# HyoKong/Cross-Resolution-Face-Recognition

Hardware: NVIDIA B200
Metric: fsrnet_train_images_per_sec (higher is better)
Workload: dtype bf16

## Files before the change

cross-resolution-face-recognition_b200/csrc/internal.h:

```cpp
#pragma once
#include <cuda_runtime.h>
#include <stddef.h>

#include "crfr.h"

#ifdef __cplusplus
#include <atomic>
#endif

enum {
  CRFR_OPT_ROWCONV_PAIR = 0,
  CRFR_OPT_WGRAD_STREAM,
  CRFR_OPT_NORM_BWD_STREAM,
  CRFR_OPT_NORM_FWD_STREAM,
  CRFR_OPT_FUSE_NORM_BWD,
  CRFR_OPT_COUNT
};
int crfr_opt(int id);

template <typename K>
inline int crfr_smem_attr(K kernel, int bytes, std::atomic<unsigned long long>& done) {
  int dev = 0;
  if (cudaGetDevice(&dev) != cudaSuccess) dev = -1;
  const unsigned long long bit = (dev >= 0 && dev < 64) ? 1ull << dev : 0ull;
// ... 18 lines not shown
  const float* rscale = nullptr;
  const float* sscale = nullptr;
};
struct crfr_pack_batch {
  crfr_pack_job job[CRFR_PACK_BATCH];
  int njobs;
};
int crfr_pack_weight_batch(const crfr_pack_job* jobs, int n, cudaStream_t st);

size_t crfr_norm_ws_bytes(int n, int hw, int c);
int crfr_norm_finalize(const float* partial, int n, int chunks, int hw, int c, float eps, float* stats,
                       cudaStream_t st);
int crfr_norm_bwd_finish(const float* partial, int chunks, const void* dsrc, int dsrc_ld, int recompute, const void* y,
                         int y_ld, const float* stats, const float* gamma, const float* beta, const float* alpha, int relu,
                         void* dy, int dy_ld, float* dgamma, float* dbeta, float* dalpha, int n, int hw, int c,
                         float* bstats, float* tot, int use_stream, cudaStream_t st);

int crfr_norm_stream_supported(int c, long long npix, const void* const* views, const int* lds, int count);
int crfr_norm_stream_parts(int n, int hw, int c);
int crfr_norm_bwd_reduce_stream(const void* da, int da_ld, const void* db, int db_ld, const void* y, int y_ld,
                                const float* stats, const float* gamma, const float* beta, const float* alpha, int relu,
                                const void* res, int res_ld, void* dz, int dz_ld, int n, int hw, int c, float* partial,
                                cudaStream_t st);
int crfr_norm_bwd_apply_stream(const void* dsrc, int dsrc_ld, int recompute, const void* y, int y_ld, const float* stats,
                               const float* partial, int parts, const float* bstats, const float* tot,
                               const float* gamma, const float* beta,
                               const float* alpha, int relu, void* dy, int dy_ld, float* dgamma, float* dbeta,
                               float* dalpha, int n, int hw, int c, cudaStream_t st);

int crfr_norm_fwd_stream(const void* y, int y_ld, const float* stats, const float* gamma, const float* beta,
                         const float* alpha, int relu, const void* res, int res_ld, void* out, int out_ld, int n, int hw,
                         int c, cudaStream_t st);

int crfr_loss_mse97_chan(const float* x, const float* t, int n, int c, int hw, float gscale, float* loss, void* dx,
                         int dx_ld, float* dchan, void* ws, size_t ws_bytes, cudaStream_t st);
int crfr_nchw_chansum(const float* g, int n, int c, int hw, float* out, void* ws, size_t ws_bytes, cudaStream_t st);

int crfr_direct_gather(int down, int n, int bh, int bw, int sh, int sw, int k, int stride, int pad, const void* src,
                       int src_ld, const void* w, int R, int s_pad, const float* bias, void* y, int y_ld,
                       float* y_nchw, cudaStream_t st);
int crfr_direct_wgrad(int n, int bh, int bw, int sh, int sw, int k, int stride, int pad, const void* small,
                      int small_ld, int A, const void* big, int big_ld, int B, float* G, void* ws, size_t ws_bytes, cudaStream_t st);
int crfr_colsum(const void* t, int ld, int c, long long npix, float* out, void* ws, size_t ws_bytes, cudaStream_t st);

struct TcGemm {
  const void* src; int n, h, w, k_total, src_ld;
  const void* wt;
  int ksize, pad, sign;
  int n_total, tile_n;
  void* out; int out_ld, out_f32;
  const float* bias;
  float* stat_ws = nullptr; size_t stat_ws_bytes = 0; int* stat_slots = nullptr;
  int stat_batch = 0;
};
int crfr_tc_gemm(const TcGemm& g, cudaStream_t st);
struct TcWgrad {
  const void* x; int n, h, w, cin, x_ld;
  const void* dy; int cout, dy_ld;
  int taps3x3;
  float* G;
  float* part = nullptr;
  size_t part_bytes = 0;
};
int crfr_tc_wgrad_raw(const TcWgrad& g, cudaStream_t st);
size_t crfr_tc_wgrad_part_bytes();

int crfr_tc_supported(int op, int h, int w, int cin, int cout, int k, int stride, int pad);
size_t crfr_tc_workspace_bytes(const crfr_conv_desc* d);
int crfr_tc_conv(const crfr_conv_desc* d, int dgrad, const void* src, const void* w_packed, const float* bias,
                 void* dst, float* stats, float eps, void* ws, size_t ws_bytes, cudaStream_t st, int batch_stats = 0);
int crfr_conv_fwd_bnstats(int engine, const crfr_conv_desc* d, const void* x, const void* w_packed, int cin_pad, void* y,
                          float* bn_stats, float eps, void* ws, size_t ws_bytes, cudaStream_t st);
int crfr_tc_wgrad(const crfr_conv_desc* d, const void* x, const void* dy, float* dw, void* ws, size_t ws_bytes,
                  cudaStream_t st);

int crfr_lowered_recipe(const crfr_conv_desc* d);
size_t crfr_lowered_ws_bytes(const crfr_conv_desc* d);
int crfr_lowered_fwd(const crfr_conv_desc* d, const void* x, const void* w_packed, int cin_pad, const float* bias,
                     void* y, float* y_nchw, void* ws, size_t ws_bytes, cudaStream_t st, float* stats = nullptr,
                     float eps = 0.f, int* stats_done = nullptr);
int crfr_lowered_dgrad(const crfr_conv_desc* d, const void* dy, const void* w_packed_t, int cout_pad, void* dx, void* ws,
                       size_t ws_bytes, cudaStream_t st);
int crfr_lowered_wgrad(const crfr_conv_desc* d, const void* x, const void* dy, float* dw, void* ws, size_t ws_bytes,
                       cudaStream_t st);
size_t crfr_lowered_dgrad_cin3_ws_bytes(const crfr_conv_desc* d);
int crfr_lowered_dgrad_cin3(const crfr_conv_desc* d, const void* dy, const void* w_packed_t, void* dx, void* ws,
                            size_t ws_bytes, cudaStream_t st);

int crfr_rowconv_supported(int h, int w, int cin, int cout, int k, int stride, int pad);
size_t crfr_rowconv_ws_bytes(int n, int h);
int crfr_rowconv_pair_supported(int n, int h);
size_t crfr_rowconv_pair_ws_bytes(int n, int h);
struct crfr_rowconv_fuse {
  const void* y; int y_ld;
  const void* db; int db_ld;
  const void* res; int res_ld;
  const float* stats; const float* gamma; const float* beta; const float* alpha; int relu;
  float* partial;
};
int crfr_rowconv_pair_parts(int n, int h, int plain = 0);
int crfr_rowconv_pair(const void* src, int src_ld, int n, int h, const void* w_packed, int flip, const float* bias,
                      void* dst, int dst_ld, float* stats, float eps, void* ws, size_t ws_bytes, cudaStream_t st,
                      const crfr_rowconv_fuse* fuse = nullptr);
int crfr_rowwgrad_supported(int h, int w, int cin, int cout, int k, int stride, int pad);
size_t crfr_rowwgrad_ws_bytes(int n, int h);
int crfr_rowwgrad(const void* x, int x_ld, const void* dy, int dy_ld, int n, int h, float* dw, void* ws,
// ... 4 lines not shown
```

cross-resolution-face-recognition_b200/csrc/lowered_conv.cu:

```cuda
#include "common.cuh"
#include "crfr.h"
#include "internal.h"

namespace {

template <int KS>
__global__ void im2col_small_kernel(const bf16* __restrict__ x, int h, int w, int oh, int ow, int stride, int pad, int sign,
                                    bf16* __restrict__ P, int kpad, int rows) {
  const int groups = kpad >> 3;
  const int idx = blockIdx.x * blockDim.x + threadIdx.x;
  if (idx >= ow * groups) return;
  const int ox = idx / groups, g = idx - ox * groups;
  const int k0 = g * 8, kmax = KS * KS * 3;
  for (int row = blockIdx.y; row < rows; row += gridDim.y) {
  const int n = row / oh, oy = row - n * oh;
  uint32_t out[4] = {0u, 0u, 0u, 0u};
  if (k0 < kmax) {
    const int t0 = k0 / 3;
    uint2 pv[4];
#pragma unroll
    for (int ti = 0; ti < 4; ++ti) {
      const int tap = t0 + ti;
      const int ky = tap / KS, kx = tap - ky * KS;
      const int y = oy * stride + sign * (ky - pad), xx = ox * stride + sign * (kx - pad);
// ... 130 lines not shown
  if (gy > (unsigned)rows) gy = (unsigned)rows;
  const dim3 grid(gx, gy);
  if (ks == 3) im2col_small_kernel<3><<<grid, 256, 0, st>>>(x, h, w, oh, ow, stride, pad, sign, P, kpad, rows);
  else if (ks == 7) im2col_small_kernel<7><<<grid, 256, 0, st>>>(x, h, w, oh, ow, stride, pad, sign, P, kpad, rows);
  else {
    crfr_set_error("im2col_small: kernel size %d not instantiated", ks);
    return CRFR_EUNSUPPORTED;
  }
  CRFR_COUNT_LAUNCH();
  CRFR_LAUNCH_CHECK();
  return CRFR_OK;
}

__global__ void col2im_small_kernel(const float* __restrict__ src, int src_ld, int C, int sh, int sw, int bh, int bw,
                                    int ks, int stride, int pad, int sgn, const float* __restrict__ bias,
                                    float* __restrict__ y_nchw, bf16* __restrict__ y, int y_ld, long long total) {
  long long i = (long long)blockIdx.x * blockDim.x + threadIdx.x;
  if (i >= total) return;
  const int X = (int)(i % bw);
  long long q = i / bw;
  const int Y = (int)(q % bh);
  const long long n = q / bh;
  float acc[4] = {0.f, 0.f, 0.f, 0.f};
#pragma unroll
  for (int c = 0; c < 4; ++c) acc[c] = (bias && c < C) ? bias[c] : 0.f;
  const int ky0 = sgn > 0 ? (Y + pad) % stride : ((pad - Y) % stride + stride) % stride;
  const int kx0 = sgn > 0 ? (X + pad) % stride : ((pad - X) % stride + stride) % stride;
  for (int ky = ky0; ky < ks; ky += stride) {
    const int ty = Y + sgn * (pad - ky);
    if (ty < 0) continue;
    const int sy = ty / stride;
    if (sy >= sh) continue;
    for (int kx = kx0; kx < ks; kx += stride) {
      const int tx = X + sgn * (pad - kx);
      if (tx < 0) continue;
      const int sx = tx / stride;
      if (sx >= sw) continue;
      const float* s = src + ((n * sh + sy) * sw + sx) * src_ld + (ky * ks + kx) * C;
#pragma unroll
      for (int c = 0; c < 4; ++c)
        if (c < C) acc[c] += s[c];
    }
  }
  if (y_nchw) {
#pragma unroll
    for (int c = 0; c < 4; ++c)
      if (c < C) y_nchw[(n * C + c) * ((long long)bh * bw) + (long long)Y * bw + X] = acc[c];
  }
  if (y) {
#pragma unroll
    for (int c = 0; c < 4; ++c)
      if (c < y_ld) y[i * y_ld + c] = __float2bfloat16_rn(c < C ? acc[c] : 0.f);
    for (int c = 4; c < y_ld; ++c) y[i * y_ld + c] = __float2bfloat16_rn(0.f);
  }
}

__global__ void __launch_bounds__(256)
col2im3_s1_kernel(const float* __restrict__ src, int h, int w, int sgn, const float* __restrict__ bias,
                  float* __restrict__ y_nchw, bf16* __restrict__ y, int y_ld) {
  constexpr int TH = 8, TW = 32, SH = TH + 2, SW = TW + 2, LD = 33;
  __shared__ float tile[SH * SW * LD];
  const int tiles_x = (w + TW - 1) / TW, tiles_y = h / TH;
  int b = blockIdx.x;
  const int tx0 = (b % tiles_x) * TW;
  b /= tiles_x;
  const int ty0 = (b % tiles_y) * TH;
  const long long n = b / tiles_y;
  const float* img = src + n * h * w * 32;
  for (int i = threadIdx.x; i < SH * SW * 8; i += 256) {
    const int px = i >> 3, q = i & 7;
    const int sy = ty0 - 1 + px / SW, sx = tx0 - 1 + px % SW;
    float4 v = make_float4(0.f, 0.f, 0.f, 0.f);
    if (sy >= 0 && sy < h && sx >= 0 && sx < w) v = *reinterpret_cast<const float4*>(img + ((long long)sy * w + sx) * 32 + q * 4);
    float* t = tile + px * LD + q * 4;
    t[0] = v.x; t[1] = v.y; t[2] = v.z; t[3] = v.w;
  }
  __syncthreads();
  const int ly = threadIdx.x >> 5, lx = threadIdx.x & 31;
  float acc[3];
#pragma unroll
  for (int c = 0; c < 3; ++c) acc[c] = bias ? bias[c] : 0.f;
#pragma unroll
  for (int ky = 0; ky < 3; ++ky)
#pragma unroll
    for (int kx = 0; kx < 3; ++kx) {
      const float* t = tile + ((ly + 1 + sgn * (1 - ky)) * SW + (lx + 1 + sgn * (1 - kx))) * LD + (ky * 3 + kx) * 3;
#pragma unroll
      for (int c = 0; c < 3; ++c) acc[c] += t[c];
    }
  const int Y = ty0 + ly, X = tx0 + lx;
  if (X >= w) return;
  if (y_nchw)
#pragma unroll
    for (int c = 0; c < 3; ++c) y_nchw[((n * 3 + c) * h + Y) * w + X] = acc[c];
  if (y) {
    const long long i = (n * h + Y) * w + X;
    for (int c = 0; c < y_ld; ++c) y[i * y_ld + c] = __float2bfloat16_rn(c < 3 ? acc[c] : 0.f);
  }
}

__device__ __forceinline__ void subpixel_of_tap(int k, int* phase, int* off) {
  const int p = (k + 2) & 3;
  *phase = p;
  *off = (p + 2 - k) / 4;
}

__global__ void deconv_subpixel_pack_kernel(const bf16* __restrict__ src, bf16* __restrict__ dst, int mode) {
  const int i = blockIdx.x * blockDim.x + threadIdx.x;
  if (i >= 49 * 64 * 64) return;
  const int s_ = i & 63, r = (i >> 6) & 63, tap = i >> 12;
  int py, dy, px, dx;
  subpixel_of_tap(tap / 7, &py, &dy);
  subpixel_of_tap(tap % 7, &px, &dx);
  const int t9 = (dy + 1) * 3 + (dx + 1), ph = py * 4 + px;
  if (mode == 0) dst[((size_t)t9 * 1024 + ph * 64 + r) * 64 + s_] = src[i];
  else dst[((size_t)t9 * 64 + r) * 1024 + ph * 64 + s_] = src[i];
}

__global__ void deconv_bias_kernel(const float* __restrict__ bias, float* __restrict__ big) {
  const int i = blockIdx.x * blockDim.x + threadIdx.x;
  if (i < 1024) big[i] = bias ? bias[i & 63] : 0.f;
}

__global__ void deconv_shuffle_kernel(bf16* __restrict__ y, int y_ld, bf16* __restrict__ all, int sh, int sw, int to_all,
                                      long long total) {
  const long long i = (long long)blockIdx.x * blockDim.x + threadIdx.x;
  if (i >= total) return;
  const int g = (int)(i & 7);
  long long p = i >> 3;
  const int X = (int)(p % (4 * sw));
  long long q = p / (4 * sw);
  const int Y = (int)(q % (4 * sh));
  const long long n = q / (4 * sh);
  const long long ai = ((n * sh + (Y >> 2)) * sw + (X >> 2)) * 1024 + ((Y & 3) * 4 + (X & 3)) * 64 + g * 8;
  uint4* py_ = reinterpret_cast<uint4*>(y + p * y_ld + g * 8);
  uint4* pa = reinterpret_cast<uint4*>(all + ai);
  if (to_all) *pa = *py_;
  else *py_ = *pa;
}

__global__ void deconv_subpixel_unpack_kernel(const float* __restrict__ G, float* __restrict__ dw) {
  const int i = blockIdx.x * blockDim.x + threadIdx.x;
  if (i >= 64 * 64 * 49) return;
  const int tap = i % 49, co = (i / 49) & 63, ci = i / (49 * 64);
  int py, dy, px, dx;
  subpixel_of_tap(tap / 7, &py, &dy);
  subpixel_of_tap(tap % 7, &px, &dx);
  const int t9 = (dy + 1) * 3 + (dx + 1), ph = py * 4 + px;
  dw[i] += G[((size_t)t9 * 64 + ci) * 1024 + ph * 64 + co];
}

__global__ void im2col_vec_kernel(const bf16* __restrict__ x, int x_ld, int C, int h, int w, int oh, int ow, int ks,
                                  int stride, int pad, bf16* __restrict__ P, long long total) {
  long long i = (long long)blockIdx.x * blockDim.x + threadIdx.x;
  if (i >= total) return;
  const int groups = C >> 3, T = ks * ks;
  const int g = (int)(i % groups);
  long long r = i / groups;
  const int tap = (int)(r % T);
  long long o = r / T;
  const int ox = (int)(o % ow);
  long long q = o / ow;
  const int oy = (int)(q % oh);
  const long long n = q / oh;
  const int ky = tap / ks, kx = tap - ky * ks;
  const int y = oy * stride + ky - pad, xx = ox * stride + kx - pad;
  uint4 v = make_uint4(0u, 0u, 0u, 0u);
  if (y >= 0 && y < h && xx >= 0 && xx < w)
    v = *reinterpret_cast<const uint4*>(x + ((n * h + y) * w + xx) * x_ld + g * 8);
// ... 217 lines not shown
      CRFR_COUNT_LAUNCH();
      CRFR_LAUNCH_CHECK();
      return CRFR_OK;
    }
    LAUNCH(col2im_small_kernel, pix, st, Q, 32, 3, d->h, d->w, d->h, d->w, 3, 1, 1, -1, bias, y_nchw, (bf16*)y,
           y ? d->out_ld : 0, pix);
    return CRFR_OK;
  }
  if (recipe == 4) {
    if (!y || y_nchw) {
      crfr_set_error("lowered conv: the transposed recipe produces the bf16 NHWC output only");
      return CRFR_EUNSUPPORTED;
    }
    const long long ipix = (long long)d->n * d->h * d->w, opix = (long long)d->n * d->oh * d->ow;
    TAKE(All, bf16, A, (size_t)ipix * 1024 * 2);
    TAKE(Wbig, bf16, A, (size_t)9 * 1024 * 64 * 2);
    TAKE(bbig, float, A, 1024 * 4);
    CRFR_CUDA(cudaMemsetAsync(Wbig, 0, (size_t)9 * 1024 * 64 * 2, st));
    LAUNCH(deconv_subpixel_pack_kernel, 49 * 64 * 64, st, (const bf16*)w_packed, Wbig, 0);
    LAUNCH(deconv_bias_kernel, 1024, st, bias, bbig);
    TcGemm g{x, d->n, d->h, d->w, 64, d->in_ld, Wbig, 3, 1, 1, 1024, 256, All, 1024, 0, bbig};
    CRFR_TRY(crfr_tc_gemm(g, st));
    LAUNCH(deconv_shuffle_kernel, opix * 8, st, (bf16*)y, d->out_ld, All, d->h, d->w, 0, opix * 8);
    return CRFR_OK;
  }
  crfr_set_error("lowered conv: no recipe for this shape");
  return CRFR_EUNSUPPORTED;
}

int crfr_lowered_dgrad(const crfr_conv_desc* d, const void* dy, const void* w_packed_t, int cout_pad, void* dx, void* ws,
                       size_t ws_bytes, cudaStream_t st) {
  const int recipe = crfr_lowered_recipe(d);
  Arena A{(uint8_t*)ws, ws_bytes, 0};
  const int T = d->k * d->k;
  if (recipe == 2) {
    const long long pix = (long long)d->n * d->h * d->w;
    TAKE(R, bf16, A, (size_t)pix * 64 * 2);
    TAKE(Wd, bf16, A, (size_t)64 * 64 * 2);
    CRFR_TRY(launch_im2col_small((const bf16*)dy, d->n, d->h, d->w, d->h, d->w, 3, 1, 1, -1, R, 64, st));
    LAUNCH(repack_tapmajor_kernel, 64 * 64, st, (const bf16*)w_packed_t, T, 64, 3, cout_pad, Wd, 64, 64);
    TcGemm g{R, d->n, d->h, d->w, 64, 64, Wd, 1, 0, 1, 64, 64, dx, d->in_ld, 0, nullptr};
    return crfr_tc_gemm(g, st);
  }
  if (recipe == 3) {
    const int kp = kpad_of(d);
    const long long opix = (long long)d->n * d->oh * d->ow, ipix = (long long)d->n * d->h * d->w;
    TAKE(dP, float, A, (size_t)opix * kp * 4);
    TAKE(Wd, bf16, A, (size_t)kp * d->cout * 2);
    CRFR_CUDA(cudaMemsetAsync(Wd, 0, (size_t)kp * d->cout * 2, st));
    CRFR_CHECK_ARG(cout_pad == d->cout, "lowered dgrad: cout_pad %d != cout %d", cout_pad, d->cout);
    CRFR_CUDA(cudaMemcpyAsync(Wd, w_packed_t, (size_t)T * 3 * d->cout * 2, cudaMemcpyDeviceToDevice, st));
    TcGemm g{dy, d->n, d->oh, d->ow, d->cout, d->out_ld, Wd, 1, 0, 1, kp, kp == 192 ? 192 : 0, dP, kp, 1, nullptr};
    CRFR_TRY(crfr_tc_gemm(g, st));
    LAUNCH(col2im_small_kernel, ipix, st, dP, kp, 3, d->oh, d->ow, d->h, d->w, d->k, d->stride, d->pad, 1, nullptr, nullptr,
           (bf16*)dx, d->in_ld, ipix);
    return CRFR_OK;
  }
  if (recipe == 5) {
    CRFR_CHECK_ARG(cout_pad == d->cout, "lowered dgrad: cout_pad %d != cout %d", cout_pad, d->cout);
    const int kc = T * d->cin;
    const long long opix = (long long)d->n * d->oh * d->ow, ipix = (long long)d->n * d->h * d->w;
    TAKE(dP, float, A, (size_t)opix * kc * 4);
    TcGemm g{dy, d->n, d->oh, d->ow, d->cout, d->out_ld, w_packed_t, 1, 0, 1, kc, 0, dP, kc, 1, nullptr};
    CRFR_TRY(crfr_tc_gemm(g, st));
    LAUNCH(col2im_vec_kernel, ipix * (d->cin / 8), st, dP, d->cin, d->oh, d->ow, d->h, d->w, d->k, d->stride, d->pad,
           (bf16*)dx, d->in_ld, ipix * (d->cin / 8));
    return CRFR_OK;
  }
  if (recipe == 4) {
    CRFR_CHECK_ARG(cout_pad == 64, "lowered dgrad: cout_pad %d != 64", cout_pad);
    const long long ipix = (long long)d->n * d->h * d->w, opix = (long long)d->n * d->oh * d->ow;
    TAKE(All, bf16, A, (size_t)ipix * 1024 * 2);
    TAKE(Wbig, bf16, A, (size_t)9 * 64 * 1024 * 2);
    LAUNCH(deconv_shuffle_kernel, opix * 8, st, (bf16*)const_cast<void*>(dy), d->out_ld, All, d->h, d->w, 1, opix * 8);
    CRFR_CUDA(cudaMemsetAsync(Wbig, 0, (size_t)9 * 64 * 1024 * 2, st));
    LAUNCH(deconv_subpixel_pack_kernel, 49 * 64 * 64, st, (const bf16*)w_packed_t, Wbig, 1);
    TcGemm g{All, d->n, d->h, d->w, 1024, 1024, Wbig, 3, 1, -1, 64, 64, dx, d->in_ld, 0, nullptr};
    return crfr_tc_gemm(g, st);
  }
  crfr_set_error("lowered dgrad: no recipe for this shape");
  return CRFR_EUNSUPPORTED;
}

size_t crfr_lowered_dgrad_cin3_ws_bytes(const crfr_conv_desc* d) {
  return (size_t)d->n * d->h * d->w * 32 * 4 + (size_t)32 * 64 * 2 + 4096;
}

int crfr_lowered_dgrad_cin3(const crfr_conv_desc* d, const void* dy, const void* w_packed_t, void* dx, void* ws,
                            size_t ws_bytes, cudaStream_t st) {
  if (crfr_lowered_recipe(d) != 1 || d->cout != 64 || d->out_ld != 64 || d->h % 8) {
    crfr_set_error("lowered dgrad (3-channel input): unsupported shape");
    return CRFR_EUNSUPPORTED;
  }
  Arena A{(uint8_t*)ws, ws_bytes, 0};
  const long long pix = (long long)d->n * d->h * d->w;
  TAKE(Q, float, A, (size_t)pix * 32 * 4);
  TAKE(Wq, bf16, A, (size_t)32 * 64 * 2);
  CRFR_CUDA(cudaMemsetAsync(Wq, 0, (size_t)32 * 64 * 2, st));
  CRFR_CUDA(cudaMemcpyAsync(Wq, w_packed_t, (size_t)27 * 64 * 2, cudaMemcpyDeviceToDevice, st));
  TcGemm g{dy, d->n, d->h, d->w, 64, d->out_ld, Wq, 1, 0, 1, 32, 32, Q, 32, 1, nullptr};
  CRFR_TRY(crfr_tc_gemm(g, st));
  col2im3_s1_kernel<<<(unsigned)(d->n * (d->h / 8) * ((d->w + 31) / 32)), 256, 0, st>>>(Q, d->h, d->w, 1, nullptr, nullptr,
                                                                                       (bf16*)dx, d->in_ld);
  CRFR_COUNT_LAUNCH();
  CRFR_LAUNCH_CHECK();
  return CRFR_OK;
}

int crfr_lowered_wgrad(const crfr_conv_desc* d, const void* x, const void* dy, float* dw, void* ws, size_t ws_bytes,
                       cudaStream_t st) {
  const int recipe = crfr_lowered_recipe(d);
  Arena A{(uint8_t*)ws, ws_bytes, 0};
  const int T = d->k * d->k;
  if (recipe == 1 || recipe == 3) {
    const int kp = kpad_of(d);
    const long long opix = (long long)d->n * d->oh * d->ow;
    TAKE(P, bf16, A, (size_t)opix * kp * 2);
    TAKE(G, float, A, (size_t)kp * d->cout * 4);
    CRFR_TRY(launch_im2col_small((const bf16*)x, d->n, d->h, d->w, d->oh, d->ow, d->k, d->stride, d->pad, 1, P, kp, st));
    CRFR_CUDA(cudaMemsetAsync(G, 0, (size_t)kp * d->cout * 4, st));
    TcWgrad g{P, d->n, d->oh, d->ow, kp, kp, dy, d->cout, d->out_ld, 0, G};
    A.rest(&g.part, &g.part_bytes);
    CRFR_TRY(crfr_tc_wgrad_raw(g, st));
    LAUNCH(unpack_lowered_kernel, (long long)d->cout * 3 * T, st, G, d->cout, dw, d->cout, 3, T, 0);
    return CRFR_OK;
  }
  if (recipe == 5) {
    const int kc = T * d->cin;
    const long long opix = (long long)d->n * d->oh * d->ow;
    TAKE(P, bf16, A, (size_t)opix * kc * 2);
// ... 38 lines not shown
```

cross-resolution-face-recognition_b200/csrc/tc_conv.cu:

```cuda
#include <cudaTypedefs.h>
#include <stdlib.h>

#include "common.cuh"
#include "crfr.h"
#include "internal.h"
#include "sm100.cuh"

using namespace sm100;

namespace {

int make_act_map(CUtensorMap* m, const void* ptr, int n, int h, int w, int c, int ld, int bw, int bh, int bn) {
  const unsigned long long dims[4] = {(unsigned long long)c, (unsigned long long)w, (unsigned long long)h,
                                      (unsigned long long)n};
  const unsigned long long strides[3] = {(unsigned long long)ld * 2, (unsigned long long)w * ld * 2,
                                         (unsigned long long)h * w * ld * 2};
  const unsigned int box[4] = {64, (unsigned int)bw, (unsigned int)bh, (unsigned int)bn};
  return crfr_tmap_encode_bf16(m, ptr, 4, dims, strides, box, "activation");
}

int make_weight_map(CUtensorMap* m, const void* ptr, long long rows, int kdim, int box_rows) {
  const unsigned long long dims[2] = {(unsigned long long)kdim, (unsigned long long)rows};
  const unsigned long long strides[1] = {(unsigned long long)kdim * 2};
  const unsigned int box[2] = {64, (unsigned int)box_rows};
  return crfr_tmap_encode_bf16(m, ptr, 2, dims, strides, box, "weights");
}

struct Tiling {
  int bw, bh, bn, tiles_x, tiles_y, tiles_n, rows;
};

bool make_tiling(int n, int h, int w, Tiling* t) {
  if (w >= 128) {
    t->bw = 128; t->bh = 1; t->bn = 1;
  } else {
    t->bw = w;
    t->bh = 128 / w;
    if (t->bh > h) t->bh = h;
    if (t->bh < 1) return false;
    t->bn = 128 / (t->bw * t->bh);
    if (t->bn < 1) t->bn = 1;
    if (t->bn > 256) return false;
  }
  t->rows = t->bw * t->bh * t->bn;
  t->tiles_x = (w + t->bw - 1) / t->bw;
  t->tiles_y = (h + t->bh - 1) / t->bh;
  t->tiles_n = (n + t->bn - 1) / t->bn;
  return t->rows <= 128 && t->rows >= 1;
}

struct ConvParams {
  int n, h, w;
  int kchunks, ksize, ntaps, pad, sign;
  int bw, bh, bn, tiles_x, tiles_y, rows;
  int total_tiles;
  int n_total;
  int out_ld;
  int out_f32;
  void* out;
  const float* bias;
  float* partial;
  int slots, gpt;
};

constexpr int kConvThreads = 192;
constexpr int kATileBytes = 128 * 128;

constexpr int kResidentIters = 9;
template <int N, int MODE = 0>
struct ConvCfg {
  static constexpr bool R = MODE == 1, T2 = MODE == 2;
  static constexpr int kBTileBytes = N * 128;
  static constexpr int kStageBytes = R ? 2 * kATileBytes : (T2 ? 2 : 1) * kATileBytes + kBTileBytes;
  static constexpr int kStages = (R || T2) ? 4 : (N <= 64) ? 8 : (N <= 128) ? 6 : 3;
  static constexpr int kAccBufs = T2 ? 4 : 2;
  static constexpr int kResidentBytes = R ? kResidentIters * kBTileBytes : 0;
  static constexpr int kTmemCols = (N <= 32) ? 32 : (N <= 64) ? 64 : (N <= 128) ? 128 : 256;
  static constexpr int kOutTiles = (N + 63) / 64;
  static constexpr int kOutBytes = kOutTiles * kATileBytes;
  static constexpr int kSmemBytes = kStages * kStageBytes + kResidentBytes + kOutBytes + 1024  + 256 ;
  static_assert(N % 32 == 0 && N <= 256 && kAccBufs * kTmemCols <= 512, "tile width");
  static_assert(kSmemBytes <= 232448, "shared memory budget");
};

template <int N, int MODE>
__global__ void __launch_bounds__(kConvThreads, 1)
tc_conv_kernel(const __grid_constant__ CUtensorMap tmA, const __grid_constant__ CUtensorMap tmB,
               const __grid_constant__ CUtensorMap tmY, ConvParams p) {
  using Cfg = ConvCfg<N, MODE>;
  constexpr bool R = Cfg::R, T2 = Cfg::T2;
  constexpr int kAB = Cfg::kAccBufs;
  extern __shared__ uint8_t smem_raw[];
  uint8_t* base = (uint8_t*)(((uintptr_t)smem_raw + 1023) & ~(uintptr_t)1023);
  uint8_t* sB = base + Cfg::kStages * Cfg::kStageBytes;
  uint8_t* sOut = sB + Cfg::kResidentBytes;
  uint64_t* full = (uint64_t*)(sOut + Cfg::kOutBytes);
  uint64_t* empty = full + Cfg::kStages;
  uint64_t* tmem_full = empty + Cfg::kStages;
  uint64_t* tmem_empty = tmem_full + kAB;
  uint64_t* w_full = tmem_empty + kAB;
  uint32_t* tmem_slot = (uint32_t*)(w_full + 1);

  const int warp = threadIdx.x >> 5, lane = threadIdx.x & 31;
  if (threadIdx.x == 0) {
    for (int s = 0; s < Cfg::kStages; ++s) {
      mbar_init(&full[s], 1);
      mbar_init(&empty[s], 1);
    }
    for (int b = 0; b < kAB; ++b) {
      mbar_init(&tmem_full[b], 1);
      mbar_init(&tmem_empty[b], 4);
    }
    mbar_init(w_full, 1);
    fence_barrier_init();
    prefetch_tmap(&tmA);
    prefetch_tmap(&tmB);
    prefetch_tmap(&tmY);
  }
  if (warp == 1) tmem_alloc<kAB * Cfg::kTmemCols>(tmem_slot);
  tc_fence_before();
  __syncthreads();
  tc_fence_after();
  const uint32_t tmem = *tmem_slot;

  const int iters = R ? 3 : p.ntaps * p.kchunks;
  const uint32_t a_bytes = (uint32_t)p.rows * 128u;
  const int ncol0 = blockIdx.y * N;
  const int my_tiles = (int)blockIdx.x < p.total_tiles ? (p.total_tiles - (int)blockIdx.x + (int)gridDim.x - 1) / (int)gridDim.x : 0;

  if (warp == 0) {
    const bool leader = elect_one();
    if (R && leader && my_tiles > 0) {
      mbar_expect_tx(w_full, (uint32_t)kResidentIters * Cfg::kBTileBytes);
      for (int tap = 0; tap < kResidentIters; ++tap)
        tma_load_2d(sB + tap * Cfg::kBTileBytes, &tmB, w_full, 0, tap * p.n_total + ncol0);
    }
    int g = 0;
    for (int i = 0; i < my_tiles; i += T2 ? 2 : 1) {
      int t = blockIdx.x + i * gridDim.x;
      const int tx = t % p.tiles_x; t /= p.tiles_x;
      const int ty = t % p.tiles_y; t /= p.tiles_y;
      const int x0 = tx * p.bw, y0 = ty * p.bh, n0 = t * p.bn;
      const bool has2 = T2 && i + 1 < my_tiles;
      int t1 = blockIdx.x + (has2 ? i + 1 : i) * gridDim.x;
      const int tx1 = t1 % p.tiles_x; t1 /= p.tiles_x;
      const int ty1 = t1 % p.tiles_y; t1 /= p.tiles_y;
      const int x1 = tx1 * p.bw, y1 = ty1 * p.bh, n1 = t1 * p.bn;
      for (int it = 0; it < iters; ++it, ++g) {
        const int s = g % Cfg::kStages;
        mbar_wait(&empty[s], ((g / Cfg::kStages) & 1) ^ 1);
        uint8_t* sa = base + s * Cfg::kStageBytes;
        if (R) {
          if (leader) {
            mbar_expect_tx(&full[s], (uint32_t)((p.bh + 2) * p.bw) * 128u);
            tma_load_4d(sa, &tmA, &full[s], 0, x0 + p.sign * (it - 1), y0 - 1, n0);
          }
          continue;
        }
        const int tap = it / p.kchunks, kc = it - tap * p.kchunks;
        const int ky = tap / p.ksize, kx = tap - ky * p.ksize;
        if (leader) {
          mbar_expect_tx(&full[s], (has2 ? 2u : 1u) * a_bytes + (uint32_t)Cfg::kBTileBytes);
          tma_load_4d(sa, &tmA, &full[s], kc * 64, x0 + p.sign * (kx - p.pad), y0 + p.sign * (ky - p.pad), n0);
          if (has2) tma_load_4d(sa + kATileBytes, &tmA, &full[s], kc * 64, x1 + p.sign * (kx - p.pad), y1 + p.sign * (ky - p.pad), n1);
          tma_load_2d(sa + (T2 ? 2 : 1) * kATileBytes, &tmB, &full[s], kc * 64, tap * p.n_total + ncol0);
        }
      }
    }
  } else if (warp == 1) {
    const bool leader = elect_one();
    const uint32_t idesc = make_idesc_bf16(128, N, 0, 0);
    const uint64_t desc0 = make_smem_desc_sw128(smem_u32(base), 16, 1024);
    const uint64_t descB = make_smem_desc_sw128(smem_u32(sB), 16, 1024);
    if (R && my_tiles > 0) mbar_wait(w_full, 0);
    int g = 0;
    for (int i = 0; i < my_tiles; i += T2 ? 2 : 1) {
      const int buf = T2 ? ((i >> 1) & 1) * 2 : (i & 1);
      const uint32_t use = T2 ? (uint32_t)(i >> 2) : (uint32_t)(i >> 1);
      mbar_wait(&tmem_empty[buf], (use & 1) ^ 1);
      if (T2) mbar_wait(&tmem_empty[buf + 1], (use & 1) ^ 1);
      tc_fence_after();
      const uint32_t d_tmem = tmem + buf * Cfg::kTmemCols;
      for (int it = 0; it < iters; ++it, ++g) {
        const int s = g % Cfg::kStages;
        mbar_wait(&full[s], (g / Cfg::kStages) & 1);
        tc_fence_after();
        const uint64_t da = desc0 + (uint64_t)((s * Cfg::kStageBytes) >> 4);
        if (R) {
          if (leader) {
#pragma unroll
            for (int ky = 0; ky < 3; ++ky) {
              const int row = p.sign > 0 ? ky : 2 - ky;
              const uint64_t dak = da + (uint64_t)((row * p.bw * 128) >> 4);
              const uint64_t dbk = descB + (uint64_t)(((ky * 3 + it) * Cfg::kBTileBytes) >> 4);
#pragma unroll
              for (int k = 0; k < 4; ++k) umma_bf16(d_tmem, dak + 2 * k, dbk + 2 * k, idesc, (uint32_t)((it | ky | k) != 0));
            }
            umma_commit(&empty[s]);
          }
          __syncwarp();
          continue;
        }
        const uint64_t db = da + (uint64_t)(((T2 ? 2 : 1) * kATileBytes) >> 4);
        if (leader) {
#pragma unroll
          for (int k = 0; k < 4; ++k) umma_bf16(d_tmem, da + 2 * k, db + 2 * k, idesc, (uint32_t)((it | k) != 0));
          if (T2 && i + 1 < my_tiles) {
            const uint64_t da1 = da + (uint64_t)(kATileBytes >> 4);
#pragma unroll
            for (int k = 0; k < 4; ++k)
              umma_bf16(d_tmem + Cfg::kTmemCols, da1 + 2 * k, db + 2 * k, idesc, (uint32_t)((it | k) != 0));
          }
// ... 264 lines not shown
    __syncwarp();
  } else if (my_tiles > 0) {
    const int q = warp & 3;
    const int r = q * 32 + lane;
    mbar_wait(tmem_full, 0);
    tc_fence_after();
    const int ci = kc * 64 + (r & 63);
    if (Cfg::kSwap) {
#pragma unroll
      const int co = N == 64 ? q * 16 + lane : r;
      const bool live = N != 64 || lane < 16;
#pragma unroll
      for (int c0 = 0; c0 < 192; c0 += 32) {
        uint32_t v[32];
        tmem_ld32(tmem + ((uint32_t)(q * 32) << 16) + c0, v);
        tmem_ld_wait();
        const int a = c0 / 64;
        const int tap = H ? a * 3 + ky : ky * 3 + a;
        float* dst = G + ((long long)tap * p.cin + kc * 64 + (c0 & 63)) * p.cout + ncol0 + co;
        if (live) {
#pragma unroll
          for (int j = 0; j < 32; ++j) dst[(long long)j * p.cout] = __uint_as_float(v[j]);
        }
      }
    } else
#pragma unroll
    for (int half = 0; half < Cfg::kAccs; ++half) {
      const int kx = half == 0 ? (r >> 6) : 2;
      const bool live = TAPS == 3 ? (half == 0 || r < 64) : (r < 64);
      const int tap = TAPS == 3 ? (H ? kx * 3 + ky : ky * 3 + kx) : 0;
      float* dst = G + ((long long)tap * p.cin + ci) * p.cout + ncol0;
#pragma unroll
      for (int c0 = 0; c0 < N; c0 += 32) {
        uint32_t v[32];
        tmem_ld32(tmem + ((uint32_t)(q * 32) << 16) + half * N + c0, v);
        tmem_ld_wait();
        if (live) {
#pragma unroll
          for (int j = 0; j < 32; j += 4)
            st_v4(dst + c0 + j, __uint_as_float(v[j]), __uint_as_float(v[j + 1]), __uint_as_float(v[j + 2]),
                  __uint_as_float(v[j + 3]));
        }
      }
    }
  }
  tc_fence_before();
  __syncthreads();
  if (warp == 1) {
    tc_fence_after();
    tmem_dealloc<Cfg::kTmemCols>(tmem);
  }
}

__global__ void wgrad_split_sum_kernel(const float4* __restrict__ part, int splits, long long slice4, float4* __restrict__ G) {
  const long long i = (long long)blockIdx.x * blockDim.x + threadIdx.x;
  if (i >= slice4) return;
  float4 s = part[i];
  for (int k = 1; k < splits; ++k) {
    const float4 v = part[k * slice4 + i];
    s.x += v.x; s.y += v.y; s.z += v.z; s.w += v.w;
  }
  G[i] = s;
}

__global__ void wgrad_unpack_kernel(const float* __restrict__ G, float* __restrict__ dw, int cin, int cout, int T) {
  long long i = (long long)blockIdx.x * blockDim.x + threadIdx.x;
  long long total = (long long)cout * cin * T;
  if (i >= total) return;
  int t = (int)(i % T);
  long long q = i / T;
  int ci = (int)(q % cin);
  int co = (int)(q / cin);
  dw[i] += G[((long long)t * cin + ci) * cout + co];
}

template <int N, int TAPS, bool H = false>
int launch_wgrad(const CUtensorMap& tmX, const CUtensorMap& tmDY, const WgradParams& p, int splits, cudaStream_t st) {
  using Cfg = WgCfg<N, TAPS, H>;
  static std::atomic<unsigned long long> attr_done{0};
  CRFR_CUDA((cudaError_t)crfr_smem_attr(tc_wgrad_kernel<N, TAPS, H>, Cfg::kSmemBytes, attr_done));
  const int gy = (TAPS == 3 ? 3 : 1) * (p.cout / N);
  tc_wgrad_kernel<N, TAPS, H><<<dim3(splits, gy, p.cin / 64), kConvThreads, Cfg::kSmemBytes, st>>>(tmX, tmDY, p);
  CRFR_COUNT_LAUNCH();
  CRFR_LAUNCH_CHECK();
  return CRFR_OK;
}

bool spatial_ok(int h, int w, bool exact128) {
  Tiling t;
  if (!make_tiling(1, h, w, &t)) return false;
  if (w > 128 && (w % 128) != 0 && exact128) return false;
  return true;
}

int pick_tile_n(int n_total) {
  const int cands[] = {256, 224, 192, 128, 96, 64, 32};
  for (int c : cands)
    if (n_total % c == 0) return c;
  return 0;
}

}

int crfr_tc_gemm(const TcGemm& g, cudaStream_t st) {
  CRFR_CHECK_ARG(((uintptr_t)g.src & 15) == 0 && ((uintptr_t)g.out & 15) == 0 && ((uintptr_t)g.wt & 15) == 0 &&
                     (g.src_ld & 7) == 0 && (g.out_ld & 3) == 0,
                 "tc_gemm: pointers must be 16B aligned and ld a multiple of 8");
  CRFR_CHECK_ARG(g.k_total % 64 == 0 && g.k_total > 0, "tc_gemm: K %d must be a multiple of 64", g.k_total);
  const int tile_n = g.tile_n ? g.tile_n : pick_tile_n(g.n_total);
  CRFR_CHECK_ARG(tile_n && g.n_total % tile_n == 0, "tc_gemm: N %d has no supported tile width", g.n_total);
  Tiling t;
  if (!make_tiling(g.n, g.h, g.w, &t)) {
    crfr_set_error("tc_gemm: unsupported spatial size %dx%d", g.h, g.w);
    return CRFR_EUNSUPPORTED;
  }
  CUtensorMap tmA, tmB, tmY;
  CRFR_TRY(make_act_map(&tmA, g.src, g.n, g.h, g.w, g.k_total, g.src_ld, t.bw, t.bh, t.bn));
  if (!g.out_f32) {
    CRFR_CHECK_ARG(tile_n % 64 == 0 && (g.out_ld & 7) == 0, "tc_gemm: bf16 output needs a tile width multiple of 64");
    CRFR_TRY(make_act_map(&tmY, g.out, g.n, g.h, g.w, g.n_total, g.out_ld, t.bw, t.bh, t.bn));
  } else {
    tmY = tmA;
  }
  const int T = g.ksize * g.ksize;
  CRFR_TRY(make_weight_map(&tmB, g.wt, (long long)T * g.n_total, g.k_total, tile_n));
  ConvParams p;
  p.n = g.n; p.h = g.h; p.w = g.w;
  p.kchunks = g.k_total / 64; p.ksize = g.ksize; p.ntaps = T; p.pad = g.pad; p.sign = g.sign;
  p.bw = t.bw; p.bh = t.bh; p.bn = t.bn; p.tiles_x = t.tiles_x; p.tiles_y = t.tiles_y; p.rows = t.rows;
  p.n_total = g.n_total; p.out_ld = g.out_ld; p.out_f32 = g.out_f32; p.out = g.out; p.bias = g.bias;
  const int tiles = t.tiles_x * t.tiles_y * t.tiles_n;
  p.total_tiles = tiles;
  p.partial = nullptr; p.slots = 0; p.gpt = 0;
  if (g.stat_slots) *g.stat_slots = 0;
  int batch_ctas = conv_sm_count() / (g.n_total / tile_n);
  if (batch_ctas > tiles) batch_ctas = tiles;
  if (batch_ctas < 1) batch_ctas = 1;
  if (g.stat_batch && g.stat_ws && g.stat_slots && !g.out_f32 && tile_n % 64 == 0 && !g.bias &&
      sizeof(float) * (size_t)batch_ctas * 4 * 2 * g.n_total <= g.stat_ws_bytes) {
    p.partial = g.stat_ws;
    p.slots = batch_ctas * 4;
    p.gpt = -1;
    *g.stat_slots = p.slots;
  } else if (g.stat_ws && g.stat_slots && !g.out_f32 && tile_n % 64 == 0 && t.rows == 128 && g.h % t.bh == 0 && g.w % t.bw == 0 &&
      (t.bw * t.bh) % 32 == 0) {
    const int area = t.bw * t.bh;
    p.gpt = area >= 128 ? 4 : area / 32;
    p.slots = t.tiles_x * t.tiles_y * p.gpt;
    if (sizeof(float) * (size_t)g.n * p.slots * 2 * g.n_total <= g.stat_ws_bytes) {
      p.partial = g.stat_ws;
      *g.stat_slots = p.slots;
    }
  }
  switch (tile_n) {
    case 32: return launch_conv<32>(tmA, tmB, tmY, p, tiles, st);
    case 64:
      if (p.ksize == 3 && p.pad == 1 && p.kchunks == 1 && p.bn == 1 && (p.bw & 7) == 0 && (p.bh + 2) * p.bw <= 256) {
        CUtensorMap tmA2;
        CRFR_TRY(make_act_map(&tmA2, g.src, g.n, g.h, g.w, g.k_total, g.src_ld, t.bw, t.bh + 2, 1));
        return launch_conv<64, 1>(tmA2, tmB, tmY, p, tiles, st);
      }
      return launch_conv<64>(tmA, tmB, tmY, p, tiles, st);
    case 96: return launch_conv<96>(tmA, tmB, tmY, p, tiles, st);
    case 128:
      if (tiles >= 4 * conv_sm_count()) return launch_conv<128, 2>(tmA, tmB, tmY, p, tiles, st);
      return launch_conv<128>(tmA, tmB, tmY, p, tiles, st);
    case 192: return launch_conv<192>(tmA, tmB, tmY, p, tiles, st);
    case 224: return launch_conv<224>(tmA, tmB, tmY, p, tiles, st);
    case 256: return launch_conv<256>(tmA, tmB, tmY, p, tiles, st);
  }
  crfr_set_error("tc_gemm: unsupported tile width %d", tile_n);
  return CRFR_EUNSUPPORTED;
}

namespace {
int launch_wgrad_any(const TcWgrad& g, const Tiling& t, const CUtensorMap& tmX, const CUtensorMap& tmDY, const WgradParams& p,
                     int splits, cudaStream_t st) {
  if (g.taps3x3) {
    if (t.bn == 1 && (t.bh + 2) * t.bw <= 256 && (g.cout == 64 || g.cout % 128 == 0)) {
      CUtensorMap tmXh;
      CRFR_TRY(make_act_map(&tmXh, g.x, g.n, g.h, g.w, g.cin, g.x_ld, t.bw, t.bh + 2, 1));
      if (g.cout == 64) return launch_wgrad<64, 3, true>(tmXh, tmDY, p, splits, st);
      return launch_wgrad<128, 3, true>(tmXh, tmDY, p, splits, st);
    }
    if (g.cout == 64) return launch_wgrad<64, 3>(tmX, tmDY, p, splits, st);
    if (g.cout % 128 == 0) return launch_wgrad<128, 3>(tmX, tmDY, p, splits, st);
    crfr_set_error("tc_wgrad: 3x3 needs cout 64 or a multiple of 128, got %d", g.cout);
    return CRFR_EUNSUPPORTED;
  }
  if (g.cout % 128 == 0) return launch_wgrad<128, 1>(tmX, tmDY, p, splits, st);
  return launch_wgrad<64, 1>(tmX, tmDY, p, splits, st);
}
}

int crfr_tc_wgrad_raw(const TcWgrad& g, cudaStream_t st) {
  CRFR_CHECK_ARG(((uintptr_t)g.x & 15) == 0 && ((uintptr_t)g.dy & 15) == 0 && (g.x_ld & 7) == 0 && (g.dy_ld & 7) == 0,
                 "tc_wgrad: pointers must be 16B aligned and ld a multiple of 8");
  CRFR_CHECK_ARG(g.cin % 64 == 0 && g.cout % 64 == 0, "tc_wgrad: channels must be multiples of 64");
  Tiling t;
  if (!make_tiling(g.n, g.h, g.w, &t)) {
    crfr_set_error("tc_wgrad: unsupported spatial size %dx%d", g.h, g.w);
    return CRFR_EUNSUPPORTED;
  }
  CUtensorMap tmX, tmDY;
  CRFR_TRY(make_act_map(&tmX, g.x, g.n, g.h, g.w, g.cin, g.x_ld, t.bw, t.bh, t.bn));
  CRFR_TRY(make_act_map(&tmDY, g.dy, g.n, g.h, g.w, g.cout, g.dy_ld, t.bw, t.bh, t.bn));
  WgradParams p;
  p.n = g.n; p.h = g.h; p.w = g.w;
  p.bw = t.bw; p.bh = t.bh; p.bn = t.bn; p.tiles_x = t.tiles_x; p.tiles_y = t.tiles_y;
  p.total_tiles = t.tiles_x * t.tiles_y * t.tiles_n;
  p.cin = g.cin; p.cout = g.cout;
  p.rows = t.rows;
  const int tile_n = (g.cout % 128 == 0) ? 128 : 64;
  const int ctas_per_split = (g.taps3x3 ? 3 : 1) * (g.cout / tile_n) * (g.cin / 64);
  const int sms = conv_sm_count();
  int splits = (2 * sms) / ctas_per_split;
  if (splits < 1) splits = ctas_per_split <= sms ? sms / ctas_per_split : 1;
  if (splits > p.total_tiles) splits = p.total_tiles;
  if (splits < 1) splits = 1;
  const long long slice = (long long)(g.taps3x3 ? 9 : 1) * g.cin * g.cout;
  const long long fit = g.part ? (long long)(g.part_bytes / (sizeof(float) * (size_t)slice)) : 0;
  if (splits > fit) splits = fit > 1 ? (int)fit : 1;
  CRFR_CHECK_ARG(splits == 1 || ((uintptr_t)g.part & 15) == 0, "tc_wgrad: partial buffer must be 16B aligned");
  p.G = splits > 1 ? g.part : g.G;
  CRFR_TRY(launch_wgrad_any(g, t, tmX, tmDY, p, splits, st));
  if (splits > 1) {
    wgrad_split_sum_kernel<<<crfr_cdiv(slice / 4, 256), 256, 0, st>>>((const float4*)g.part, splits, slice / 4, (float4*)g.G);
    CRFR_COUNT_LAUNCH();
    CRFR_LAUNCH_CHECK();
  }
  return CRFR_OK;
}

size_t crfr_tc_wgrad_part_bytes() {
  return sizeof(float) * (size_t)2 * conv_sm_count() * 3 * 64 * 128 + 256;
}

int crfr_tc_supported(int op, int h, int w, int cin, int cout, int k, int stride, int pad) {
  if (k != 3 || stride != 1 || pad != 1) return 0;
  if (cin % 64 || cout % 64) return 0;
  const int nout = (op == 1) ? cin : cout;
  if (op == 2) {
    if (cout != 64 && cout % 128 != 0) return 0;
    return spatial_ok(h, w, true) ? 1 : 0;
  }
  if (pick_tile_n(nout) == 0) return 0;
  return spatial_ok(h, w, false) ? 1 : 0;
}

size_t crfr_tc_workspace_bytes(const crfr_conv_desc* d) {
  size_t wg = sizeof(float) * (size_t)d->k * d->k * d->cin * d->cout + 256 + crfr_tc_wgrad_part_bytes();
  {
    Tiling t;
    if (make_tiling(d->n, d->oh, d->ow, &t)) {
      const size_t sp = sizeof(float) * (size_t)d->n * t.tiles_x * t.tiles_y * 4 * 2 * d->cout + 256;
      if (sp > wg) wg = sp;
    }
  }
  if (crfr_rowconv_supported(d->h, d->w, d->cin, d->cout, d->k, d->stride, d->pad)) {
    const size_t rc = crfr_rowconv_ws_bytes(d->n, d->h);
    if (rc > wg) wg = rc;
    const size_t rw = crfr_rowwgrad_ws_bytes(d->n, d->h);
    if (rw > wg) wg = rw;
  }
  return wg;
}

int crfr_tc_conv(const crfr_conv_desc* d, int dgrad, const void* src, const void* w_packed, const float* bias,
                 void* dst, float* stats, float eps, void* ws, size_t ws_bytes, cudaStream_t st, int batch_stats) {
  if (!batch_stats && crfr_rowconv_supported(d->h, d->w, d->cin, d->cout, d->k, d->stride, d->pad)) {
    return crfr_rowconv(src, dgrad ? d->out_ld : d->in_ld, d->n, d->h, w_packed, dgrad, bias, dst,
                        dgrad ? d->in_ld : d->out_ld, dgrad ? nullptr : stats, eps, ws, ws_bytes, st);
  }
  TcGemm g;
  g.src = src; g.n = d->n; g.h = d->h; g.w = d->w;
  g.k_total = dgrad ? d->cout : d->cin;
  g.src_ld = dgrad ? d->out_ld : d->in_ld;
  g.wt = w_packed; g.ksize = d->k; g.pad = d->pad; g.sign = dgrad ? -1 : 1;
  g.n_total = dgrad ? d->cin : d->cout;
  g.tile_n = g.n_total <= 256 ? g.n_total : 0;
// ... 43 lines not shown
```

Before: 3450.

## Skip zero K-steps in subpixel deconv, add s4 col2im, rework split-sum

Adds a list of nonzero (tap, phase) K-steps so the subpixel deconvolution GEMM only iterates over the 49 nonzero weight blocks instead of all 144. It also adds a specialized shared-memory col2im kernel for 7x7 stride-4 dgrad with 3 output channels, replacing the generic col2im_small path. The wgrad split-sum kernel is rewritten to use scalar loads with batched independent loads across splits and smaller blocks for more memory-level parallelism. The step list is passed by value in the kernel parameters, which enlarges the parameter block.

```diff
diff --git a/cross-resolution-face-recognition_b200/csrc/internal.h b/cross-resolution-face-recognition_b200/csrc/internal.h
--- a/cross-resolution-face-recognition_b200/csrc/internal.h
+++ b/cross-resolution-face-recognition_b200/csrc/internal.h
@@ -94,6 +94,7 @@
   const float* bias;
   float* stat_ws = nullptr; size_t stat_ws_bytes = 0; int* stat_slots = nullptr;
   int stat_batch = 0;
+  const unsigned char* steps = nullptr; int nsteps = 0;
 };
 int crfr_tc_gemm(const TcGemm& g, cudaStream_t st);
 struct TcWgrad {
diff --git a/cross-resolution-face-recognition_b200/csrc/lowered_conv.cu b/cross-resolution-face-recognition_b200/csrc/lowered_conv.cu
--- a/cross-resolution-face-recognition_b200/csrc/lowered_conv.cu
+++ b/cross-resolution-face-recognition_b200/csrc/lowered_conv.cu
@@ -206,6 +206,59 @@
     for (int c = 0; c < 4; ++c)
       if (c < y_ld) y[i * y_ld + c] = __float2bfloat16_rn(c < C ? acc[c] : 0.f);
     for (int c = 4; c < y_ld; ++c) y[i * y_ld + c] = __float2bfloat16_rn(0.f);
+  }
+}
+
+constexpr int kS4Lo = 64, kS4Hi = 89;
+__global__ void __launch_bounds__(512)
+col2im7_s4_kernel(const float* __restrict__ dP, int ld, int sh, int sw, bf16* __restrict__ y, int y_ld) {
+  extern __shared__ float s4[];
+  float* lo = s4;
+  float* hi = s4 + sw * kS4Lo;
+  const int a = blockIdx.x % sh;
+  const long long n = blockIdx.x / sh;
+  const float4* rhi = reinterpret_cast<const float4*>(dP + ((n * sh + a) * sw) * (long long)ld);
+  for (int i = threadIdx.x; i < sw * 22; i += blockDim.x) {
+    const int sx = i / 22, j = i - sx * 22;
+    const float4 v = rhi[(sx * ld >> 2) + 15 + j];
+    float* t = hi + sx * kS4Hi + 4 * j;
+    t[0] = v.x; t[1] = v.y; t[2] = v.z; t[3] = v.w;
+  }
+  const bool has_lo = a + 1 < sh;
+  if (has_lo) {
+    const float4* rlo = rhi + (sw * ld >> 2);
+    for (int i = threadIdx.x; i < sw * 16; i += blockDim.x) {
+      const int sx = i >> 4, j = i & 15;
+      reinterpret_cast<float4*>(lo + sx * kS4Lo)[j] = rlo[(sx * ld >> 2) + j];
+    }
+  }
+  __syncthreads();
+  const int w = 4 * sw;
+  for (int i = threadIdx.x; i < 4 * w; i += blockDim.x) {
+    const int r = i / w, X = i - r * w, b = X >> 2, s = X & 3;
+    float acc[3] = {0.f, 0.f, 0.f};
+#pragma unroll
+    for (int hy = 0; hy < 2; ++hy) {
+      if (hy == 0 && (r == 0 || !has_lo)) continue;
+      const float* rowp = hy == 0 ? lo : hi;
+      const int ldr = hy == 0 ? kS4Lo : kS4Hi, off = hy == 0 ? 0 : 60;
+      const int ky = hy == 0 ? r - 1 : r + 3;
+#pragma unroll
+      for (int hx = 0; hx < 2; ++hx) {
+        if (hx == 0 && (s == 0 || b + 1 >= sw)) continue;
+        const int sx = hx == 0 ? b + 1 : b, kx = hx == 0 ? s - 1 : s + 3;
+        const float* t = rowp + sx * ldr + (ky * 7 + kx) * 3 - off;
+#pragma unroll
+        for (int c = 0; c < 3; ++c) acc[c] += t[c];
+      }
+    }
+    const long long p = ((n * 4 * sh) + 4 * a + r) * (long long)w + X;
+    if (y_ld == 4) {
+      const __nv_bfloat162 c01 = __floats2bfloat162_rn(acc[0], acc[1]), c2z = __floats2bfloat162_rn(acc[2], 0.f);
+      *reinterpret_cast<uint2*>(y + p * 4) = make_uint2(*reinterpret_cast<const uint32_t*>(&c01), *reinterpret_cast<const uint32_t*>(&c2z));
+    } else {
+      for (int c = 0; c < y_ld; ++c) y[p * y_ld + c] = __float2bfloat16_rn(c < 3 ? acc[c] : 0.f);
+    }
   }
 }
 
@@ -269,6 +322,19 @@
   const int t9 = (dy + 1) * 3 + (dx + 1), ph = py * 4 + px;
   if (mode == 0) dst[((size_t)t9 * 1024 + ph * 64 + r) * 64 + s_] = src[i];
   else dst[((size_t)t9 * 64 + r) * 1024 + ph * 64 + s_] = src[i];
+}
+
+int deconv_nonzero_steps(unsigned char* steps) {
+  bool nz[9 * 16] = {};
+  for (int ky = 0; ky < 7; ++ky)
+    for (int kx = 0; kx < 7; ++kx) {
+      const int py = (ky + 2) & 3, dy = (py + 2 - ky) / 4, px = (kx + 2) & 3, dx = (px + 2 - kx) / 4;
+      nz[((dy + 1) * 3 + (dx + 1)) * 16 + py * 4 + px] = true;
+    }
+  int n = 0;
+  for (int i = 0; i < 9 * 16; ++i)
+    if (nz[i]) steps[n++] = (unsigned char)i;
+  return n;
 }
 
 __global__ void deconv_bias_kernel(const float* __restrict__ bias, float* __restrict__ big) {
@@ -592,6 +658,13 @@
     CRFR_CUDA(cudaMemcpyAsync(Wd, w_packed_t, (size_t)T * 3 * d->cout * 2, cudaMemcpyDeviceToDevice, st));
     TcGemm g{dy, d->n, d->oh, d->ow, d->cout, d->out_ld, Wd, 1, 0, 1, kp, kp == 192 ? 192 : 0, dP, kp, 1, nullptr};
     CRFR_TRY(crfr_tc_gemm(g, st));
+    if (d->k == 7 && d->stride == 4 && d->h == 4 * d->oh && d->w == 4 * d->ow && d->ow <= 64) {
+      col2im7_s4_kernel<<<(unsigned)(d->n * d->oh), 512, (size_t)d->ow * (kS4Lo + kS4Hi) * sizeof(float), st>>>(
+          dP, kp, d->oh, d->ow, (bf16*)dx, d->in_ld);
+      CRFR_COUNT_LAUNCH();
+      CRFR_LAUNCH_CHECK();
+      return CRFR_OK;
+    }
     LAUNCH(col2im_small_kernel, ipix, st, dP, kp, 3, d->oh, d->ow, d->h, d->w, d->k, d->stride, d->pad, 1, nullptr, nullptr,
            (bf16*)dx, d->in_ld, ipix);
     return CRFR_OK;
@@ -616,6 +689,9 @@
     CRFR_CUDA(cudaMemsetAsync(Wbig, 0, (size_t)9 * 64 * 1024 * 2, st));
     LAUNCH(deconv_subpixel_pack_kernel, 49 * 64 * 64, st, (const bf16*)w_packed_t, Wbig, 1);
     TcGemm g{All, d->n, d->h, d->w, 1024, 1024, Wbig, 3, 1, -1, 64, 64, dx, d->in_ld, 0, nullptr};
+    unsigned char steps[49];
+    g.steps = steps;
+    g.nsteps = deconv_nonzero_steps(steps);
     return crfr_tc_gemm(g, st);
   }
   crfr_set_error("lowered dgrad: no recipe for this shape");
diff --git a/cross-resolution-face-recognition_b200/csrc/tc_conv.cu b/cross-resolution-face-recognition_b200/csrc/tc_conv.cu
--- a/cross-resolution-face-recognition_b200/csrc/tc_conv.cu
+++ b/cross-resolution-face-recognition_b200/csrc/tc_conv.cu
@@ -49,6 +49,7 @@
   return t->rows <= 128 && t->rows >= 1;
 }
 
+constexpr int kMaxListedSteps = 160;
 struct ConvParams {
   int n, h, w;
   int kchunks, ksize, ntaps, pad, sign;
@@ -61,6 +62,8 @@
   const float* bias;
   float* partial;
   int slots, gpt;
+  int nsteps;
+  unsigned char steps[kMaxListedSteps];
 };
 
 constexpr int kConvThreads = 192;
@@ -123,7 +126,7 @@
   tc_fence_after();
   const uint32_t tmem = *tmem_slot;
 
-  const int iters = R ? 3 : p.ntaps * p.kchunks;
+  const int iters = R ? 3 : (p.nsteps ? p.nsteps : p.ntaps * p.kchunks);
   const uint32_t a_bytes = (uint32_t)p.rows * 128u;
   const int ncol0 = blockIdx.y * N;
   const int my_tiles = (int)blockIdx.x < p.total_tiles ? (p.total_tiles - (int)blockIdx.x + (int)gridDim.x - 1) / (int)gridDim.x : 0;
@@ -157,7 +160,8 @@
           }
           continue;
         }
-        const int tap = it / p.kchunks, kc = it - tap * p.kchunks;
+        const int code = p.nsteps ? (int)p.steps[it] : it;
+        const int tap = code / p.kchunks, kc = code - tap * p.kchunks;
         const int ky = tap / p.ksize, kx = tap - ky * p.ksize;
         if (leader) {
           mbar_expect_tx(&full[s], (has2 ? 2u : 1u) * a_bytes + (uint32_t)Cfg::kBTileBytes);
@@ -528,14 +532,22 @@
   }
 }
 
-__global__ void wgrad_split_sum_kernel(const float4* __restrict__ part, int splits, long long slice4, float4* __restrict__ G) {
+constexpr int kSplitSumThreads = 64, kSplitSumBatch = 16;
+__global__ void __launch_bounds__(kSplitSumThreads)
+wgrad_split_sum_kernel(const float* __restrict__ part, int splits, long long slice, float* __restrict__ G) {
   const long long i = (long long)blockIdx.x * blockDim.x + threadIdx.x;
-  if (i >= slice4) return;
-  float4 s = part[i];
-  for (int k = 1; k < splits; ++k) {
-    const float4 v = part[k * slice4 + i];
-    s.x += v.x; s.y += v.y; s.z += v.z; s.w += v.w;
-  }
+  if (i >= slice) return;
+  const float* src = part + i;
+  float s = src[0];
+  int k = 1;
+  for (; k + kSplitSumBatch <= splits; k += kSplitSumBatch) {
+    float v[kSplitSumBatch];
+#pragma unroll
+    for (int j = 0; j < kSplitSumBatch; ++j) v[j] = src[(long long)(k + j) * slice];
+#pragma unroll
+    for (int j = 0; j < kSplitSumBatch; ++j) s += v[j];
+  }
+  for (; k < splits; ++k) s += src[(long long)k * slice];
   G[i] = s;
 }
 
@@ -608,6 +620,13 @@
   const int tiles = t.tiles_x * t.tiles_y * t.tiles_n;
   p.total_tiles = tiles;
   p.partial = nullptr; p.slots = 0; p.gpt = 0;
+  CRFR_CHECK_ARG(g.nsteps >= 0 && g.nsteps <= kMaxListedSteps && g.nsteps <= T * p.kchunks && (g.nsteps == 0 || g.steps),
+                 "tc_gemm: %d listed K steps", g.nsteps);
+  p.nsteps = g.nsteps;
+  for (int i = 0; i < g.nsteps; ++i) {
+    CRFR_CHECK_ARG(g.steps[i] < T * p.kchunks, "tc_gemm: listed K step %d out of range", (int)g.steps[i]);
+    p.steps[i] = g.steps[i];
+  }
   if (g.stat_slots) *g.stat_slots = 0;
   int batch_ctas = conv_sm_count() / (g.n_total / tile_n);
   if (batch_ctas > tiles) batch_ctas = tiles;
@@ -631,7 +650,7 @@
   switch (tile_n) {
     case 32: return launch_conv<32>(tmA, tmB, tmY, p, tiles, st);
     case 64:
-      if (p.ksize == 3 && p.pad == 1 && p.kchunks == 1 && p.bn == 1 && (p.bw & 7) == 0 && (p.bh + 2) * p.bw <= 256) {
+      if (p.ksize == 3 && p.pad == 1 && p.kchunks == 1 && !p.nsteps && p.bn == 1 && (p.bw & 7) == 0 && (p.bh + 2) * p.bw <= 256) {
         CUtensorMap tmA2;
         CRFR_TRY(make_act_map(&tmA2, g.src, g.n, g.h, g.w, g.k_total, g.src_ld, t.bw, t.bh + 2, 1));
         return launch_conv<64, 1>(tmA2, tmB, tmY, p, tiles, st);
@@ -701,7 +720,7 @@
   p.G = splits > 1 ? g.part : g.G;
   CRFR_TRY(launch_wgrad_any(g, t, tmX, tmDY, p, splits, st));
   if (splits > 1) {
-    wgrad_split_sum_kernel<<<crfr_cdiv(slice / 4, 256), 256, 0, st>>>((const float4*)g.part, splits, slice / 4, (float4*)g.G);
+    wgrad_split_sum_kernel<<<crfr_cdiv(slice, kSplitSumThreads), kSplitSumThreads, 0, st>>>(g.part, splits, slice, g.G);
     CRFR_COUNT_LAUNCH();
     CRFR_LAUNCH_CHECK();
   }
```

New measurement: 3482 (median of 6 runs). About the same (+0.9%).
